# rossumur/espflix

Measured on AMD Instinct MI355X. Metric: MPEG-1 352x192 frames/s, higher is better.
Workload: dtype u8/int32; 1 GPU; 1024 streams/GPU x GOP(12) I+11P, 352x192 MPEG-1 ES resident in HBM, ids rank*1024.. per rank (BASELINE configs[2]; at 8 GPUs = configs[4], stream k on rank floor(k*8/8192)); streams_per_gpu=1024, streams_total=1024, es_bytes_per_gpu=46457181, parallelism=stream-partition x1, coefficients_per_gpu=44531885, ring_depth=2

## Files before the change

espflix_amd/csrc/efx_api.hip:

```cpp
#include <hip/hip_runtime.h>

#include <algorithm>
#include <memory>
#include <mutex>
#include <thread>

#include <cstdio>
#include <cstdlib>
#include <cstring>
#include <string>
#include <vector>

#include "efx.h"
#include "efx_internal.h"
#include "enc_core.h"
#include "parse_tm.h"

namespace efx {
struct DemuxChunk;
__global__ void k_demux_scan(const uint8_t*, const uint64_t*, const uint32_t*, const uint32_t*, DemuxChunk*);
__global__ void k_demux_offsets(const uint32_t*, const uint32_t*, DemuxChunk*, uint8_t*, const uint64_t*, uint32_t*, uint32_t*);
__global__ void k_demux(const uint8_t*, const uint64_t*, const uint32_t*, const uint32_t*, const DemuxChunk*, uint8_t*, PesEntry*);
__global__ void k_demux_fused(const uint8_t*, const uint64_t*, const uint32_t*, const uint32_t*, DemuxChunk*, uint8_t*, PesEntry*, uint32_t*, uint32_t*,
                              uint32_t*);
__global__ void k_demux_audio_scan(const uint8_t*, const uint64_t*, const uint32_t*, const uint32_t*, DemuxChunk*);
__global__ void k_demux_audio_offsets(const uint32_t*, const uint32_t*, DemuxChunk*, uint32_t*);
__global__ void k_demux_audio(const uint8_t*, const uint64_t*, const uint32_t*, const uint32_t*, const DemuxChunk*, uint8_t*, const uint64_t*);
__global__ void k_ts_sequences(const uint8_t*, const uint64_t*, const uint32_t*, const uint32_t*, PesEntry*, IdxInfo*);
__global__ void k_idx_bins(const PesEntry*, const uint32_t*, const IdxInfo*, uint32_t, uint32_t*, size_t);
__global__ void k_index(const uint8_t*, const uint64_t*, int, PicInfo*, SliceTmp*, uint32_t*, uint32_t*, uint32_t*,
                        const uint32_t*, const PesEntry*, const uint32_t*, const uint32_t*, int64_t*, int64_t*, int, int, int);
__global__ void k_advance(StreamState*, const uint32_t*, int64_t*, const int64_t*, int, int, int, int32_t*);
__global__ void k_slice_scan(const PicInfo*, const uint32_t*, int, int, const uint32_t*, uint32_t*, DecodeCounters*);
__global__ void k_slice_emit(const PicInfo*, const SliceTmp*, const uint32_t*, const uint64_t*, const uint32_t*, int, int,
                             const uint32_t*, SliceDesc*, uint32_t*);
__global__ void k_parse(const uint8_t*, const SliceDesc*, DecodeCounters*, const TmTables*, MbRec*, TmU4*, uint32_t*, uint32_t*,
                        int, int);
__global__ void k_recon(const MbRec*, const uint32_t*, const uint32_t*, const uint32_t*, uint8_t*, int, int, int, const int32_t*, int, int);
__global__ void k_recon_all(const MbRec*, const uint32_t*, const uint32_t*, const uint32_t*, uint8_t*, int, int, int, const int32_t*, int, int,
                            int, uint32_t*, uint32_t*, int);

__global__ void k_frame_hash(const uint8_t*, int, uint64_t*);
__global__ void k_fill(uint32_t*, uint32_t, size_t);
__global__ void k_composite(const uint8_t*, const VideoTables*, const VideoLineTemplates*, FieldArgs, uint16_t*);
__global__ void k_pdm(const int16_t*, int, int, int32_t*, uint16_t*);
template <int FMT, int CHROMA>
__global__ void k_export(const uint8_t*, int, ExportArgs);
__global__ void k_enc_begin(EncArgs);
__global__ void k_enc_rows(EncArgs);
__global__ void k_enc_pack(EncArgs);
__global__ void k_sbc(const uint8_t*, size_t, int, int, SbcState*, const SbcTables*, int16_t*, size_t, uint32_t*, uint32_t*, int);
__global__ void k_sbc_frames(const uint8_t*, size_t, int, int, SbcFrameInfo*, uint32_t*, uint32_t*, SbcQueues*);
__global__ void k_sbc_plan(const SbcFrameInfo*, int, int, const SbcState*, SbcFramePlan*, uint32_t*, SbcQueues*, uint32_t*, int, int, uint32_t*,
                           uint32_t*, SbcExtraItem*, uint8_t*);
__global__ void k_sbc_par_stereo(const uint8_t*, size_t, int, int, const SbcState*, SbcState*, const SbcTables*, const SbcFrameInfo*, int16_t*,
                                 size_t, uint32_t*, int, SbcQueues*, const uint32_t*, int, const SbcExtraItem*, int);
__global__ void k_sbc_par_mono(const uint8_t*, size_t, int, int, const SbcState*, SbcState*, const SbcTables*, const SbcFrameInfo*, int16_t*,
                               size_t, uint32_t*, int, SbcQueues*, const uint32_t*, int, const SbcExtraItem*, int);
__global__ void k_sbc_gen(const uint8_t*, size_t, int, int, const SbcState*, SbcState*, const SbcTables*, const SbcFrameInfo*,
                          const SbcFramePlan*, int16_t*, size_t, int, SbcQueues*, const uint32_t*, int, const uint8_t*, int);
__global__ void k_sbc_finish(const uint8_t*, size_t, int, int, SbcState*, const SbcState*, const SbcTables*, int16_t*, size_t, uint32_t*,
                             uint32_t*, int, uint32_t*);
}

using namespace efx;

#ifndef EFX_SBC_WG_PER_CU
#define EFX_SBC_WG_PER_CU 4
#endif

#ifndef EFX_PARSE_STREAMS
#define EFX_PARSE_STREAMS 2
#endif
#ifndef EFX_SLOTS
#define EFX_SLOTS 3
#endif
constexpr int kParseStreams = EFX_PARSE_STREAMS;
constexpr int kMaxGroups = 16;
static_assert(kMaxGroups <= kExportMaxGroups, "k_export takes every reconstruction group of a call");
#ifndef EFX_RECON_MERGE
#define EFX_RECON_MERGE 1
#endif
constexpr int kReconMerge = EFX_RECON_MERGE;
#ifndef EFX_GROUP_STREAMS
#define EFX_GROUP_STREAMS 1024
#endif
// ... 19 lines not shown
    uint8_t* d_frames = nullptr;
    StreamState* d_state = nullptr;

    struct Upload {
        uint8_t* d_es = nullptr;
        uint64_t* d_stream_off = nullptr;
        uint32_t* d_stream_perm = nullptr;
        uint32_t* d_ts_len = nullptr;
        uint32_t* d_pkt_base = nullptr;
        uint32_t* d_es_len = nullptr;
        uint32_t* d_pes_count = nullptr;
        PesEntry* d_pes = nullptr;
        uint8_t* h_es = nullptr;
        uint8_t* h_meta = nullptr;
        std::vector<uint64_t> stream_off;
        std::vector<uint32_t> es_len;
        int n_streams = 0;
        int sort_groups = 1;
        size_t es_used = 0, ts_bytes = 0;
        bool ts_input = false, valid = false;
        hipEvent_t uploaded = nullptr;
        hipEvent_t last_read[kParseStreams] = {};
        hipEvent_t ev_demux[2] = {nullptr, nullptr};
        bool demux_timed = false;
    } up[kUploads];
    int cur_up = -1;
    struct Arena {
        uint8_t* base;
        size_t bytes;
        bool owned;
    };
    std::vector<Arena> arenas;
    hipStream_t copy_stream = nullptr;
    uint8_t* d_ts = nullptr;
    DemuxChunk* d_demux_chunks = nullptr;
    size_t pes_cap = 0;
    IdxInfo* d_idx_info = nullptr;
    uint64_t* d_ts_off = nullptr;
    uint32_t* d_idx_len = nullptr;
    uint32_t* d_idx_base = nullptr;
    PesEntry* d_idx_seq = nullptr;
    bool ts_ready = false;

    struct Slot {
        uint32_t* d_pic_count = nullptr;
        uint32_t* d_status = nullptr;
        DecodeCounters* d_counters = nullptr;
        MbRec* d_mbrecs = nullptr;
        TmU4* d_raw = nullptr;
        uint32_t* d_coefs = nullptr;
        PicInfo* d_pics = nullptr;
        SliceTmp* d_slices_tmp = nullptr;
        uint32_t* d_qtab = nullptr;
        uint32_t* d_slice_base = nullptr;
        SliceDesc* d_descs = nullptr;
        int64_t* d_pts = nullptr;
        int32_t* d_call_pos = nullptr;
        uint32_t* d_recon_sync = nullptr;
        hipEvent_t parse_done[kReconMerge] = {}, recon_done = nullptr, wrap_cleared = nullptr;
        int epoch = 0;
        int upload = 0;
    } slot[kSlots];
    struct TimingEvents {
        hipEvent_t ev[5] = {nullptr, nullptr, nullptr, nullptr, nullptr};
    };
    std::vector<TimingEvents> timing_ring;
    uint64_t timed_calls = 0;
    struct Group {
        int slot, first, count;
        int half0, halves;
    };
    Group groups[kMaxGroups];
    int n_groups = 0;
    hipEvent_t last_recon_done = nullptr;
    uint64_t recon_groups_unsynced = 0;
    int last_upload = 0;
    int last_n_streams = 0;
    bool last_ts_input = false;
    uint64_t subcalls = 0;
    uint64_t parse_calls = 0;
    uint8_t timing_groups[kTimingRing] = {};
    uint16_t timing_launches[kTimingRing] = {};
    uint16_t timing_leaders[kTimingRing] = {};
    hipStream_t parse_streams[kParseStreams] = {};
    VideoTables* d_video[2] = {nullptr, nullptr};
    VideoLineTemplates* d_video_lines[2] = {nullptr, nullptr};
    SbcTables* d_sbc_tables = nullptr;
    int parse_wg_cap = 0;
    int opt_groups = 0;
    int opt_parse_cap = 0;
    int opt_recon_mode = 0;
    int opt_recon_waves = 0;
    int opt_recon_items = 16;
    int n_cus = 256;
    uint32_t* d_sbc_flags = nullptr;
    SbcState* d_sbc_next = nullptr;
    size_t sbc_flags_cap = 0;
    SbcFrameInfo* d_sbc_info = nullptr;
    SbcFramePlan* d_sbc_plan = nullptr;
    SbcExtraItem* d_sbc_extra = nullptr;
    uint8_t* d_sbc_cover = nullptr;
    size_t sbc_info_cap = 0;
    size_t sbc_gran_cap = 0;
    int opt_sbc_serial = 0;
    int opt_demux_fused = 0;
    bool sbc_flags_clean = false;
    uint64_t* d_hash = nullptr;
// ... 256 lines not shown
        int lo = 0, hi = 0;
        if (hipDeviceGetStreamPriorityRange(&lo, &hi) != hipSuccess)
            return bail(EFX_ERR_DEVICE);
        for (auto& ps : ctx->parse_streams)
            if (hipStreamCreateWithPriority(&ps, hipStreamNonBlocking, hi) != hipSuccess)
                return bail(EFX_ERR_DEVICE);
        if (hipStreamCreateWithFlags(&ctx->copy_stream, hipStreamNonBlocking) != hipSuccess)
            return bail(EFX_ERR_DEVICE);
        std::vector<hipStream_t> order = {ctx->stream};
        for (auto ps : ctx->parse_streams)
            order.push_back(ps);
        order.push_back(ctx->copy_stream);
        for (hipStream_t st : order) {
            hipLaunchKernelGGL(k_fill, dim3(1), dim3(64), 0, st, (uint32_t*)nullptr, 0u, (size_t)0);
            if (hipStreamSynchronize(st) != hipSuccess)
                return bail(EFX_ERR_DEVICE);
        }
    }
    const size_t n = (size_t)cfg->max_streams, P = (size_t)cfg->max_pictures, D = (size_t)ctx->cfg.ring_depth;
    ctx->es_cap = ctx->cfg.max_stream_bytes + n * (kEsTailBytes + 32) + kEsGuardBytes;
    ctx->es_cap = (ctx->es_cap + 255) & ~(size_t)255;
    if (ctx->es_cap * kCoefsPerEsByte >= 0xFFFFFFFFull)
        return bail(EFX_ERR_CAPACITY);
    hipError_t e = hipSuccess;
    auto A = [&](hipError_t r) {
        if (e == hipSuccess)
            e = r;
    };
    A(dalloc(&ctx->d_tables, 1));
    A(dalloc(&ctx->d_tm_tables, 1));
    A(dalloc(&ctx->d_state, n));
    for (auto& u : ctx->up) {
        A(dalloc(&u.d_es, ctx->es_cap));
        A(dalloc(&u.d_stream_off, n + 1));
        A(dalloc(&u.d_stream_perm, n));
        A(hipHostMalloc(reinterpret_cast<void**>(&u.h_es), ctx->es_cap, hipHostMallocDefault));
        A(hipHostMalloc(reinterpret_cast<void**>(&u.h_meta), meta_bytes(n), hipHostMallocDefault));
        A(hipEventCreateWithFlags(&u.uploaded, hipEventDisableTiming));
        for (auto& ev : u.last_read)
            A(hipEventCreateWithFlags(&ev, hipEventDisableTiming));
        if (e == hipSuccess)
            A(hipMemset(u.d_es, 0, ctx->es_cap));
    }
    for (auto& sl : ctx->slot) {
        A(dalloc(&sl.d_pic_count, n));
        A(dalloc(&sl.d_status, n));
        A(dalloc(&sl.d_counters, kMaxGroups));
        A(dalloc(&sl.d_mbrecs, n * P * kMbCount));
        A(dalloc(&sl.d_raw, n * P * kMbCount));
        A(dalloc(&sl.d_coefs, ctx->es_cap * kCoefsPerEsByte));
        A(dalloc(&sl.d_pics, n * P));
        A(dalloc(&sl.d_slices_tmp, n * P * kMaxSlicesPerPicture));
        A(dalloc(&sl.d_qtab, n * P * 64));
        A(dalloc(&sl.d_slice_base, n * P + kMaxGroups));
        A(dalloc(&sl.d_descs, n * P * kMaxSlicesPerPicture));
        A(dalloc(&sl.d_call_pos, 2 * n));
        A(dalloc(&sl.d_recon_sync, kReconSyncWords(n)));
    }
    A(dalloc(&ctx->d_frames, n * D * kFrameBytes + 8192));
    A(dalloc(&ctx->d_video[0], 1));
    A(dalloc(&ctx->d_video[1], 1));
    A(dalloc(&ctx->d_video_lines[0], 1));
    A(dalloc(&ctx->d_video_lines[1], 1));
    A(dalloc(&ctx->d_hash, n * D));
    A(dalloc(&ctx->d_sbc_tables, 1));
    if (e != hipSuccess) {
        fprintf(stderr, "efx_create: %s\n", hipGetErrorString(e));
        return bail(EFX_ERR_DEVICE);
    }
    {
        hipDeviceProp_t prop;
        if (hipGetDeviceProperties(&prop, cfg->device) == hipSuccess) {
            ctx->parse_wg_cap = std::max(1, prop.multiProcessorCount * 5 / 8);
            ctx->n_cus = std::max(1, prop.multiProcessorCount);
        }
        if (const char* v = getenv("EFX_GROUPS"))
            ctx->opt_groups = atoi(v);
        if (const char* v = getenv("EFX_FORCE_PARSE_CAP"))
            ctx->opt_parse_cap = atoi(v);
        if (const char* v = getenv("EFX_RECON_MODE"))
            ctx->opt_recon_mode = atoi(v);
        if (const char* v = getenv("EFX_RECON_WAVES"))
            ctx->opt_recon_waves = atoi(v);
        if (const char* v = getenv("EFX_DEMUX_FUSED"))
            ctx->opt_demux_fused = atoi(v) != 0;
        if (const char* v = getenv("EFX_RECON_ITEMS"))
            ctx->opt_recon_items = atoi(v);
        if (const char* cap = getenv("EFX_PARSE_WG_CAP"))
            ctx->parse_wg_cap = atoi(cap);
    }
    ParseTables* pt = new ParseTables;
    build_parse_tables(pt);
    A(hipMemcpy(ctx->d_tables, pt, sizeof(ParseTables), hipMemcpyHostToDevice));
    {
        TmTables* tt = new TmTables;
        build_tm_tables(tt);
        hipError_t e_tm = hipMemcpy(ctx->d_tm_tables, tt, sizeof(TmTables), hipMemcpyHostToDevice);
        delete tt;
        A(e_tm);
    }
    delete pt;
    for (int ntsc = 0; ntsc < 2; ntsc++) {
        VideoTables vt;
        build_video_tables(ntsc, &vt);
        A(hipMemcpy(ctx->d_video[ntsc], &vt, sizeof(vt), hipMemcpyHostToDevice));
        VideoLineTemplates* lt = new VideoLineTemplates;
        build_video_line_templates(&vt, lt);
// ... 23 lines not shown
    return EFX_OK;
}

void efx_destroy(efx_ctx* ctx)
{
    bind_device(ctx);
    if (!ctx)
        return;
    if (ctx->copy_stream)
        (void)hipStreamSynchronize(ctx->copy_stream);
    for (auto ps : ctx->parse_streams)
        if (ps)
            (void)hipStreamSynchronize(ps);
    if (ctx->stream)
        (void)hipStreamSynchronize(ctx->stream);
    for (auto& a : ctx->arenas) {
        if (a.owned)
            (void)hipHostFree(a.base);
        else
            (void)hipHostUnregister(a.base);
    }
    void* bufs[] = {ctx->d_tables, ctx->d_tm_tables, ctx->d_sbc_flags, ctx->d_sbc_next, ctx->d_sbc_info, ctx->d_sbc_plan, ctx->d_sbc_extra, ctx->d_sbc_cover, ctx->d_state, ctx->d_frames, ctx->d_video[0],  ctx->d_video[1], ctx->d_video_lines[0],
                    ctx->d_video_lines[1], ctx->d_hash, ctx->d_ts, ctx->d_demux_chunks, ctx->d_sbc_tables, ctx->d_idx_info, ctx->d_ts_off, ctx->d_idx_len,
                    ctx->d_idx_base, ctx->d_idx_seq, ctx->d_enc_state, ctx->d_enc_pics, ctx->d_enc_slices, ctx->d_enc_slice_len,
                    ctx->d_enc_tables};
    if (ctx->h_enc_full)
        (void)hipHostFree(ctx->h_enc_full);
    for (auto& te : ctx->timing_ring)
        for (auto& ev : te.ev)
            if (ev)
                (void)hipEventDestroy(ev);
    for (void* b : bufs)
        if (b)
            (void)dev_free(b);
    for (auto& u : ctx->up) {
        void* ub[] = {u.d_es, u.d_stream_off, u.d_stream_perm, u.d_ts_len, u.d_pkt_base, u.d_es_len, u.d_pes_count, u.d_pes};
        for (void* b : ub)
            if (b)
                (void)dev_free(b);
        if (u.h_es)
            (void)hipHostFree(u.h_es);
        if (u.h_meta)
            (void)hipHostFree(u.h_meta);
        hipEvent_t evs[] = {u.uploaded, u.ev_demux[0], u.ev_demux[1]};
        for (auto ev : evs)
            if (ev)
                (void)hipEventDestroy(ev);
        for (auto ev : u.last_read)
            if (ev)
                (void)hipEventDestroy(ev);
    }
    for (auto& sl : ctx->slot) {
        void* sb[] = {sl.d_pic_count, sl.d_status, sl.d_counters, sl.d_mbrecs, sl.d_raw, sl.d_coefs, sl.d_pts, sl.d_call_pos, sl.d_recon_sync,
                      sl.d_pics,      sl.d_slices_tmp, sl.d_qtab, sl.d_slice_base, sl.d_descs};
        for (void* b : sb)
            if (b)
                (void)dev_free(b);
        for (auto ev : sl.parse_done)
            if (ev)
                (void)hipEventDestroy(ev);
        if (sl.recon_done)
            (void)hipEventDestroy(sl.recon_done);
        if (sl.wrap_cleared)
            (void)hipEventDestroy(sl.wrap_cleared);
    }
    bool complete = ctx->own_stream && ctx->stream && ctx->copy_stream;
    for (auto ps : ctx->parse_streams)
        complete = complete && ps;
    if (ctx->pooled_streams && complete) {
        StreamSet set;
        set.recon = ctx->stream;
        for (int i = 0; i < kParseStreams; i++)
            set.parse[i] = ctx->parse_streams[i];
        set.copy = ctx->copy_stream;
        set.serial = ctx->stream_serial;
        park_stream_set(ctx->cfg.device, set);
    } else {
        for (auto ps : ctx->parse_streams)
            if (ps)
                (void)hipStreamDestroy(ps);
        if (ctx->copy_stream)
            (void)hipStreamDestroy(ctx->copy_stream);
        if (ctx->own_stream && ctx->stream)
            (void)hipStreamDestroy(ctx->stream);
    }
    delete ctx;
}


static int ensure_ts_buffers(efx_ctx* ctx)
{
    if (ctx->ts_ready)
        return EFX_OK;
    if (ctx->d_ts)
        return fail(ctx, EFX_ERR_DEVICE, "transport-stream buffers: an earlier allocation failed");
    const size_t n_max = (size_t)ctx->cfg.max_streams;
    ctx->pes_cap = ctx->es_cap / 188 + n_max;
    hipError_t e = dalloc(&ctx->d_ts, ctx->es_cap);
    if (e == hipSuccess)
        e = dev_alloc(reinterpret_cast<void**>(&ctx->d_demux_chunks), (ctx->pes_cap / kDemuxChunk + n_max + 2) * 16 + n_max * sizeof(uint32_t));
    for (auto& u : ctx->up) {
        if (e == hipSuccess) e = dalloc(&u.d_ts_len, n_max);
        if (e == hipSuccess) e = dalloc(&u.d_pkt_base, n_max);
        if (e == hipSuccess) e = dalloc(&u.d_es_len, n_max);
        if (e == hipSuccess) e = dalloc(&u.d_pes_count, n_max);
        if (e == hipSuccess) e = dalloc(&u.d_pes, ctx->pes_cap);
        for (auto& ev : u.ev_demux)
// ... 454 lines not shown
                                      : (idle_at_call ? group_count(n_all) : 1);
    {
        bool nested = true;
        for (int g = 1; g < G && nested; g++) {
            bool found = false;
            for (int k = 0; k <= u.sort_groups && !found; k++)
                found = group_first(n_all, u.sort_groups, k) == group_first(n_all, G, g);
            nested = found;
        }
        if (!nested) {
            int r = sync_all(ctx);
            if (r)
                return r;
            std::vector<uint32_t> perm((size_t)n_all);
            for (int i = 0; i < n_all; i++)
                perm[i] = (uint32_t)i;
            auto len_of = [&](uint32_t i) { return u.stream_off[i + 1] - u.stream_off[i]; };
            for (int g = 0; g < G; g++)
                std::stable_sort(perm.begin() + group_first(n_all, G, g), perm.begin() + group_first(n_all, G, g + 1),
                                 [&](uint32_t a, uint32_t b) { return len_of(a) > len_of(b); });
            EFX_HIP(hipMemcpy(u.d_stream_perm, perm.data(), perm.size() * sizeof(uint32_t), hipMemcpyHostToDevice));
            u.sort_groups = G;
        }
    }
    hipStream_t sr = ctx->stream;
    int timing_slot = -1;
    if (ctx->timing && !ctx->timing_ring.empty()) {
        timing_slot = (int)(ctx->timed_calls++ % kTimingRing);
        ctx->timing_groups[timing_slot] = (uint8_t)G;
        ctx->timing_leaders[timing_slot] = 0;
        ctx->timing_launches[timing_slot] = (uint16_t)(((G + kReconMerge - 1) / kReconMerge) * (ctx->opt_recon_mode == 0 ? n_pictures : 1));
    }
    ctx->last_upload = ctx->cur_up;
    ctx->last_n_streams = u.n_streams;
    ctx->last_ts_input = u.ts_input;
    const int R = (G + kReconMerge - 1) / kReconMerge;
    ctx->n_groups = R;
    for (int r = 0; r < R; r++) {
        const int h0 = r * kReconMerge, h1 = std::min(G, h0 + kReconMerge);
        const int rs0 = group_first(n_all, G, h0), rn = group_first(n_all, G, h1) - rs0;
        const int slot = (int)(ctx->subcalls++ % kSlots);
        ctx->groups[r] = {slot, rs0, rn, h0, h1 - h0};
        efx_ctx::Slot& sl = ctx->slot[slot];
        sl.upload = ctx->cur_up;
        const bool wrap = ++sl.epoch > 255;
        if (wrap)
            sl.epoch = 1;
        efx_ctx::TimingEvents* te0 = nullptr;
        for (int g = h0; g < h1; g++) {
            const int s0 = group_first(n_all, G, g), n = group_first(n_all, G, g + 1) - s0;
            const int pi = (int)(ctx->parse_calls++ % kParseStreams);
            hipStream_t sp = ctx->parse_streams[pi];
            DecodeCounters* counters = sl.d_counters + g;
            uint32_t* slice_base = sl.d_slice_base + (size_t)s0 * P + g;
            SliceDesc* descs = sl.d_descs + (size_t)s0 * P * kMaxSlicesPerPicture;

            EFX_HIP(hipStreamWaitEvent(sp, u.uploaded, 0));
            EFX_HIP(hipStreamWaitEvent(sp, sl.recon_done, 0));
            if (wrap && g == h0) {
                EFX_HIP(hipMemsetAsync(sl.d_mbrecs, 0, (size_t)ctx->cfg.max_streams * P * kMbCount * sizeof(MbRec), sp));
                EFX_HIP(hipEventRecord(sl.wrap_cleared, sp));
            } else if (wrap)
                EFX_HIP(hipStreamWaitEvent(sp, sl.wrap_cleared, 0));
            efx_ctx::TimingEvents* te = timing_slot >= 0 ? &ctx->timing_ring[(size_t)timing_slot * kMaxGroups + g] : nullptr;
            if (te && !te->ev[0])
                for (auto& ev : te->ev)
                    EFX_HIP(hipEventCreate(&ev));
            if (g == h0)
                te0 = te;
            if (te)
                EFX_HIP(hipEventRecord(te->ev[0], sp));
            hipLaunchKernelGGL(k_index, dim3(n), dim3(64 * kIndexWaves), 0, sp, u.d_es, u.d_stream_off, P, sl.d_pics, sl.d_slices_tmp,
                               sl.d_pic_count, sl.d_status, sl.d_qtab, ctx->d_tables->scan, u.d_pes, u.d_pkt_base, u.d_pes_count,
                               u.ts_input ? sl.d_pts : nullptr, u.ts_input ? sl.d_pts + (size_t)ctx->cfg.max_streams * P : nullptr,
                               first_picture, s0, n_pictures);
            hipLaunchKernelGGL(k_slice_scan, dim3(1), dim3(1024), 0, sp, sl.d_pics, sl.d_pic_count, n, P, u.d_stream_perm + s0,
                               slice_base, counters);
            hipLaunchKernelGGL(k_slice_emit, dim3((n * P * kMaxSlicesPerPicture + 255) / 256), dim3(256), 0, sp, sl.d_pics,
                               sl.d_slices_tmp, sl.d_pic_count, u.d_stream_off, slice_base, n, P, u.d_stream_perm + s0, descs, sl.d_status);
            if (te)
                EFX_HIP(hipEventRecord(te->ev[1], sp));
            const int max_slices = n * P * kMaxSlicesPerPicture;
            const int parse_waves = (max_slices + kParseLanes - 1) / kParseLanes;
            int parse_wgs = (parse_waves + kParseWaves - 1) / kParseWaves;
            const bool recon_busy = ctx->opt_parse_cap == 1 || (ctx->opt_parse_cap == 0 && ctx->recon_groups_unsynced > 0);
            if (ctx->parse_wg_cap > 0 && recon_busy)
                parse_wgs = std::min(parse_wgs, ctx->parse_wg_cap);
            hipLaunchKernelGGL(k_parse, dim3(parse_wgs), dim3(64 * kParseWaves), 0, sp, u.d_es,
                               descs, counters, ctx->d_tm_tables, sl.d_mbrecs, sl.d_raw, sl.d_coefs, sl.d_status, P, sl.epoch);
            if (te)
                EFX_HIP(hipEventRecord(te->ev[2], sp));
            EFX_HIP(hipEventRecord(sl.parse_done[g - h0], sp));
            EFX_HIP(hipEventRecord(u.last_read[pi], sp));
        }

        for (int g = h0; g < h1; g++)
            EFX_HIP(hipStreamWaitEvent(sr, sl.parse_done[g - h0], 0));
        if (te0) {
            EFX_HIP(hipEventRecord(te0->ev[4], sr));
            ctx->timing_leaders[timing_slot] |= (uint16_t)(1u << h0);
        }
        hipLaunchKernelGGL(k_advance, dim3((rn + 255) / 256), dim3(256), 0, sr, ctx->d_state, sl.d_pic_count,
                           u.ts_input ? sl.d_pts : nullptr, u.ts_input ? sl.d_pts + (size_t)ctx->cfg.max_streams * P : nullptr, rs0, rn,
                           P, sl.d_call_pos);
        constexpr int kGroupsPerPicture = (kMbCount * 6 + 63) / 64;
#ifdef EFX_RECON_ITEMS2
        constexpr int kReconGridY = (kGroupsPerPicture + 1) / 2;
#else
        constexpr int kReconGridY = kGroupsPerPicture;
#endif
        if (ctx->opt_recon_mode == 0) {
            for (int p = 0; p < n_pictures; p++)
                hipLaunchKernelGGL(k_recon, dim3(rn, kReconGridY), dim3(64), 0, sr, sl.d_mbrecs, sl.d_coefs,
                                   ctx->d_tables->scan, sl.d_qtab, ctx->d_frames, P, D, p, sl.d_call_pos, sl.epoch, rs0);
        } else if (rn > 0) {
            EFX_HIP(hipMemsetAsync(sl.d_recon_sync, 0, kReconSyncWords((size_t)rn) * sizeof(uint32_t), sr));
            const long long items = (long long)rn * kGroupsPerPicture * n_pictures;
            const int per_cu = ctx->opt_recon_waves > 0 ? ctx->opt_recon_waves : 18;
            const long long waves = ctx->opt_recon_items > 0 ? (items + ctx->opt_recon_items - 1) / ctx->opt_recon_items
                                                             : std::min<long long>(items, (long long)ctx->n_cus * per_cu);
            hipLaunchKernelGGL(k_recon_all, dim3((unsigned)waves), dim3(64), 0, sr, sl.d_mbrecs,
                               sl.d_coefs, ctx->d_tables->scan, sl.d_qtab, ctx->d_frames, P, D, n_pictures, sl.d_call_pos, sl.epoch, rs0, rn,
                               sl.d_recon_sync, sl.d_status, ctx->opt_recon_items);
        }
        if (te0)
            EFX_HIP(hipEventRecord(te0->ev[3], sr));
        EFX_HIP(hipEventRecord(sl.recon_done, sr));
        ctx->last_recon_done = sl.recon_done;
        ctx->recon_groups_unsynced++;
    }
    EFX_HIP(hipGetLastError());
    ctx->decoded = true;
// ... 787 lines not shown
            float a = 0, b = 0, c = 0;
            EFX_HIP(hipEventElapsedTime(&a, te.ev[0], te.ev[1]));
            EFX_HIP(hipEventElapsedTime(&b, te.ev[1], te.ev[2]));
            if (leaders >> g & 1) {
                EFX_HIP(hipEventElapsedTime(&c, te.ev[4], te.ev[3]));
                last_leader = g;
                n_leaders++;
            }
            t.index_ms += a / n_timed;
            t.parse_ms += b / n_timed;
            t.recon_ms += c / n_timed;
        }
        float d = 0;
        EFX_HIP(hipEventElapsedTime(&d, ctx->timing_ring[call * kMaxGroups].ev[0], ctx->timing_ring[call * kMaxGroups + last_leader].ev[3]));
        t.total_ms += d / n_timed;
        if (k == 0) {
            t.groups = (uint32_t)n_leaders;
            t.parse_halves = (uint32_t)G;
            t.recon_launches = ctx->timing_launches[call];
        } else if (t.groups != (uint32_t)n_leaders || t.parse_halves != (uint32_t)G || t.recon_launches != ctx->timing_launches[call])
            t.mixed = 1;
    }
    t.timed_calls = (uint32_t)n_timed;
    for (int i = 0; i < ctx->n_streams; i++)
        t.pictures += ctx->h_pic_count[i];
    t.slices = ctx->h_counters.total_slices;
    t.coefficients = ctx->h_counters.coefficients;
    {
        efx_ctx::Upload& u = ctx->up[ctx->last_upload];
        t.es_bytes = u.es_used;
        t.ts_bytes = u.ts_bytes;
        if (u.ts_input && u.demux_timed)
            EFX_HIP(hipEventElapsedTime(&t.demux_ms, u.ev_demux[0], u.ev_demux[1]));
    }
    *out = t;
    return EFX_OK;
}


int efx_debug_poke(efx_ctx* ctx, void* dptr, size_t bytes, long long offset_bytes)
{
    bind_device(ctx);
    if (!ctx || !dptr)
        return EFX_ERR_ARG;
    (void)bytes;
    char* at = static_cast<char*>(dptr) + offset_bytes;
    hipLaunchKernelGGL(k_fill, dim3(1), dim3(64), 0, ctx->stream, reinterpret_cast<uint32_t*>(at), 0xDEADBEEFu, (size_t)1);
    EFX_HIP(hipGetLastError());
    EFX_HIP(hipStreamSynchronize(ctx->stream));
    ctx->recon_groups_unsynced = 0;
    return EFX_OK;
}

int efx_debug_recon_stats(efx_ctx* ctx, uint32_t out[64])
{
    bind_device(ctx);
    if (!ctx || !out || !ctx->decoded || ctx->n_groups < 1)
        return EFX_ERR_ARG;
    int r = sync_all(ctx);
    if (r)
        return r;
    std::vector<uint32_t> all(64 * 32);
    EFX_HIP(hipMemcpy(all.data(), ctx->slot[ctx->groups[ctx->n_groups - 1].slot].d_recon_sync, all.size() * sizeof(uint32_t), hipMemcpyDeviceToHost));
    for (int k = 0; k < 64; k++)
        out[k] = all[(size_t)k * 32];
    return EFX_OK;
}

int efx_device_alloc(efx_ctx* ctx, size_t bytes, void** dptr)
{
    bind_device(ctx);
    if (!ctx || !dptr)
        return EFX_ERR_ARG;
    EFX_HIP(dev_alloc(dptr, bytes));
    return EFX_OK;
}

int efx_device_free(efx_ctx* ctx, void* dptr)
{
    bind_device(ctx);
    if (!ctx)
        return EFX_ERR_ARG;
    EFX_HIP(dev_free(dptr));
    return EFX_OK;
}

int efx_memcpy_h2d(efx_ctx* ctx, void* dst_device, const void* src, size_t bytes)
{
    bind_device(ctx);
    if (!ctx || !dst_device || !src)
        return EFX_ERR_ARG;
    EFX_HIP(hipStreamSynchronize(ctx->stream));
    ctx->recon_groups_unsynced = 0;
    EFX_HIP(hipMemcpy(dst_device, src, bytes, hipMemcpyHostToDevice));
    return EFX_OK;
}

int efx_memcpy_d2h(efx_ctx* ctx, void* dst, const void* src_device, size_t bytes)
{
    bind_device(ctx);
    if (!ctx || !dst || !src_device)
        return EFX_ERR_ARG;
    EFX_HIP(hipStreamSynchronize(ctx->stream));
    ctx->recon_groups_unsynced = 0;
    EFX_HIP(hipMemcpy(dst, src_device, bytes, hipMemcpyDeviceToHost));
    return EFX_OK;
// ... 4 lines not shown
```

espflix_amd/csrc/efx_internal.h:

```cpp
#pragma once
#include <cstdint>

namespace efx {

constexpr int kMbW = 22, kMbH = 12, kMbCount = 264;
constexpr int kStride = 528, kStripBytes = 8448, kFrameBytes = 101376;
constexpr int kMaxSlicesPerPicture = 16;
#ifndef EFX_PARSE_LANES
#define EFX_PARSE_LANES 64
#endif
constexpr int kParseLanes = EFX_PARSE_LANES;
#ifndef EFX_PARSE_WAVES
#define EFX_PARSE_WAVES 4
#endif
constexpr int kParseWaves = EFX_PARSE_WAVES;
constexpr int kIndexWaves = 4;
constexpr int kMaxUnitsPerStream = 4096;
constexpr int kCoefsPerEsByte = 4;
constexpr int kEsTailBytes = 9;
constexpr int kEsGuardBytes = 512;

struct PicInfo {
    uint32_t first_slice;
    uint16_t n_slices;
    uint8_t type;
    uint8_t full_pel;
    uint8_t r_size;
    uint8_t custom_q;
    uint16_t reserved;
    uint32_t seq_off;
    uint32_t start_off;
};

struct PesEntry {
    uint32_t es_off;
    uint32_t reserved;
    int64_t pts;
};

struct StreamState {
    uint32_t fb_index;
    uint32_t pts_seen;
    int64_t pts_carry;
};

constexpr int64_t kNoPts = INT64_MIN;

struct SliceTmp {
    uint32_t off;
    uint32_t len_code;
};

struct SliceDesc {
    uint32_t es_off;
    uint32_t es_len;
    uint32_t stream;
    uint32_t pic_code_flags;
    uint32_t mb_limit;
    uint32_t reserved;
};
// ... 170 lines not shown
```

espflix_amd/csrc/k_index.hip:

```cpp
#include <hip/hip_runtime.h>

#include "efx_internal.h"
#include "efx.h"

namespace efx {

namespace {

__device__ inline uint32_t wave_excl_scan(uint32_t v, uint32_t* total)
{
    uint32_t x = v;
    int lane = threadIdx.x & 63;
#pragma unroll
    for (int d = 1; d < 64; d <<= 1) {
        uint32_t y = __shfl_up(x, d, 64);
        if (lane >= d)
            x += y;
    }
    *total = __shfl(x, 63, 64);
    return x - v;
}

__device__ inline uint32_t load_bits(const uint8_t* p, uint32_t bitpos, int n)
{
// ... 316 lines not shown
            }
            pts_out[(size_t)s * max_pictures + p] = a ? mp[a - 1].pts : -1;
        }
    }

    for (uint32_t p = wave; p < npics; p += kIndexWaves) {
        PicInfo pi = mypics[p];
        if (!pi.custom_q)
            continue;
        uint32_t flags = pi.reserved;
        const uint8_t* sp = base + pi.seq_off;
        uint32_t intra_bit = 63, non_intra_bit = (flags & 1) ? 64 + 512 : 64;
        uint32_t t = scan_tab[lane];
        uint32_t zz = t & 0xFF;
        uint32_t qi = (flags & 1) ? load_bits(sp, intra_bit + 8 * zz, 8) : ((t >> 16) & 0xFF);
        uint32_t qn = (flags & 2) ? load_bits(sp, non_intra_bit + 8 * zz, 8) : 16;
        qtab[((size_t)s * max_pictures + p) * 64 + lane] = (t & 0xFFFF) | (qi << 16) | (qn << 24);
    }
}

__global__ void k_advance(StreamState* __restrict__ state, const uint32_t* __restrict__ pic_count, int64_t* __restrict__ pts,
                          const int64_t* __restrict__ pts_newest, int stream0, int n_streams, int max_pictures,
                          int32_t* __restrict__ call_pos)
{
    const int t = blockIdx.x * blockDim.x + threadIdx.x;
    if (t >= n_streams)
        return;
    const int s = stream0 + t;
    StreamState st = state[s];
    const int n = (int)pic_count[s];
    int f = st.pts_seen ? -1 : n;
    if (pts) {
        int64_t* my = pts + (size_t)s * max_pictures;
        for (int i = 0; i < n; i++) {
            if (my[i] == -1 && st.pts_carry != -1)
                my[i] = st.pts_carry;
            if (f == n && my[i] != -1)
                f = i;
        }
        if (pts_newest[s] != kNoPts)
            st.pts_carry = pts_newest[s];
    } else if (!st.pts_seen)
        f = 0;
    call_pos[2 * s] = (int32_t)st.fb_index;
    call_pos[2 * s + 1] = f;
    if (n > 0) {
        st.fb_index += f < 0 ? (uint32_t)n : (uint32_t)(n - 1 > f ? n - 1 - f : 0);
        if (f < n)
            st.pts_seen = 1;
    }
    state[s] = st;
}

__global__ __launch_bounds__(1024) void k_slice_scan(const PicInfo* __restrict__ pics,
                                                     const uint32_t* __restrict__ pic_count, int n_streams,
                                                     int max_pictures, const uint32_t* __restrict__ stream_perm,
                                                     uint32_t* __restrict__ slice_base,
                                                     DecodeCounters* __restrict__ counters)
{
    __shared__ uint32_t wave_tot[16];
    __shared__ uint32_t carry;
    constexpr int kRun = 4;
    const int tid = threadIdx.x, lane = tid & 63, wv = tid >> 6;
    const int n = n_streams * max_pictures;
    if (tid == 0)
        carry = 0;
    __syncthreads();
    for (int base = 0; base < n; base += 1024 * kRun) {
        uint32_t v[kRun];
#pragma unroll
        for (int r = 0; r < kRun; r++) {
            const int i = base + tid * kRun + r;
            v[r] = 0;
            if (i < n) {
                int p = i / n_streams, s = (int)stream_perm[i - p * n_streams];
                if ((uint32_t)p < pic_count[s])
                    v[r] = pics[(size_t)s * max_pictures + p].n_slices;
            }
        }
        uint32_t mine = 0;
#pragma unroll
        for (int r = 0; r < kRun; r++)
            mine += v[r];
        uint32_t tot;
        uint32_t ex = wave_excl_scan(mine, &tot);
        if (lane == 63)
            wave_tot[wv] = tot;
        __syncthreads();
        uint32_t off = carry;
        for (int k = 0; k < wv; k++)
            off += wave_tot[k];
        uint32_t at = off + ex;
#pragma unroll
        for (int r = 0; r < kRun; r++) {
            const int i = base + tid * kRun + r;
            if (i < n)
                slice_base[i] = at;
            at += v[r];
        }
        __syncthreads();
        if (tid == 1023)
            carry = at;
        __syncthreads();
    }
    if (tid == 0) {
        counters->total_slices = carry;
        counters->streams = (uint32_t)n_streams;
        counters->coefficients = 0;
        counters->macroblocks = 0;
        counters->next_wave = 0;
        slice_base[n] = carry;
    }
}

__global__ __launch_bounds__(256) void k_slice_emit(const PicInfo* __restrict__ pics,
                                                    const SliceTmp* __restrict__ slices_tmp,
                                                    const uint32_t* __restrict__ pic_count,
                                                    const uint64_t* __restrict__ stream_off,
                                                    const uint32_t* __restrict__ slice_base, int n_streams,
                                                    int max_pictures, const uint32_t* __restrict__ stream_perm,
                                                    SliceDesc* __restrict__ descs, uint32_t* __restrict__ status)
{
    int t = blockIdx.x * blockDim.x + threadIdx.x;
    int k = t % kMaxSlicesPerPicture, i = t / kMaxSlicesPerPicture;
    if (i >= n_streams * max_pictures)
        return;
    int p = i / n_streams, s = (int)stream_perm[i - p * n_streams];
    if ((uint32_t)p >= pic_count[s])
        return;
    PicInfo pi = pics[(size_t)s * max_pictures + p];
    if (k >= pi.n_slices)
        return;
    SliceTmp st = slices_tmp[(size_t)s * max_pictures * kMaxSlicesPerPicture + pi.first_slice + k];
    SliceDesc d;
    d.es_off = (uint32_t)stream_off[s] + st.off;
    d.es_len = st.len_code >> 8;
    d.stream = (uint32_t)s;
    d.pic_code_flags = (uint32_t)p | ((st.len_code & 0xFF) << 8) | ((uint32_t)pi.type << 16) | ((uint32_t)pi.full_pel << 18) |
                       ((uint32_t)pi.r_size << 19) | ((uint32_t)pi.custom_q << 22);
    uint32_t limit = kMbCount;
    bool out_of_order = false;
    {
        const uint32_t code = st.len_code & 0xFF;
        const SliceTmp* all = slices_tmp + (size_t)s * max_pictures * kMaxSlicesPerPicture + pi.first_slice;
        for (int j = 0; j < (int)pi.n_slices; j++) {
            const uint32_t other = all[j].len_code & 0xFF;
            if (other > code && (other - 1) * kMbW < limit)
                limit = (other - 1) * kMbW;
            if (other == code && j > k)
                limit = 0;
            out_of_order |= j < k && other >= code;
        }
    }
    if (out_of_order)
        atomicOr(&status[s], EFX_STREAM_SLICE_ORDER);
    d.mb_limit = limit;
    d.reserved = 0;
    descs[slice_base[i] + k] = d;
}

}
```

espflix_amd/csrc/k_parse.hip:

```cpp
#include <hip/hip_runtime.h>

#include "efx_internal.h"
#include "efx.h"
#include "parse_tm.h"
#include "efx_probe.h"

namespace efx {

namespace {

constexpr int kRingDwords = 16;
#ifndef EFX_TRIPS_PER_TOPUP
#define EFX_TRIPS_PER_TOPUP 4
#endif
constexpr int kTripsPerTopup = EFX_TRIPS_PER_TOPUP;
constexpr int kRingLow = kTripsPerTopup + 4;
#ifndef EFX_DRAIN_WORDS
#define EFX_DRAIN_WORDS 4
#endif
constexpr int kDrainWords = EFX_DRAIN_WORDS;
constexpr int kStageWords = (kTripsPerTopup <= 4 && kDrainWords == 4) ? 8 : 16;

struct BitReader {
    const uint4* gp;
// ... 123 lines not shown
__device__ __forceinline__ void parse_group(uint32_t w, const uint8_t* __restrict__ es, const SliceDesc* __restrict__ descs,
                                            DecodeCounters* __restrict__ counters, SharedTables& sh, MbRec* __restrict__ mbrecs,
                                            TmU4* __restrict__ raw_recs, uint32_t* __restrict__ coefs, uint32_t* __restrict__ status,
                                            int max_pictures, int epoch)
{
    const uint32_t gid = w * kParseLanes + (threadIdx.x & 63);
    const bool mine = (threadIdx.x & 63) < kParseLanes && gid < counters->total_slices;
    SliceDesc d = {};
    if (mine)
        d = descs[gid];
    const uint32_t pic = d.pic_code_flags & 0xFF;
    EFX_PROBE_CLAIM(1, w);
    EFX_PROBE_STAMP(1);
    const int code = (d.pic_code_flags >> 8) & 0xFF;
    const int first_mb = (code - 1) * kMbW;
    const int mb_limit = (int)d.mb_limit;
    const bool has_slice = mine && mb_limit > first_mb;

    TmSlice sp;
    sp.coef_last = (d.es_off + d.es_len) * kCoefsPerEsByte - 1;
    sp.type_bit = ((d.pic_code_flags >> 16) & 3) == 1 ? kTmTypeIBit : 0u;
    sp.r_size = (d.pic_code_flags >> 19) & 7;
    sp.max_mbs = has_slice ? (uint32_t)(mb_limit - first_mb) : 0u;
    const size_t rec0 = ((size_t)d.stream * max_pictures + pic) * kMbCount;
    TmU4* const raw = raw_recs + rec0 + (has_slice ? first_mb : 0);

    BitReader br;
    br.init(es, d.es_off, &sh.ring[threadIdx.x >> 6][0][threadIdx.x & 63]);

    TmFix fx;
    {
        fx.qscale = br.window() >> 27;
        br.advance(5);
        while (has_slice && (br.window() >> 31)) {
            br.advance(9);
            br.topup();
        }
        br.advance(1);
    }
    TmLane L;
    const uint32_t tok_base = d.es_off * kCoefsPerEsByte;
    tm_begin(L, tok_base, has_slice);
    auto store_raw = [&](uint32_t k, uint32_t a, uint32_t b, uint32_t c, uint32_t e) { raw[k] = make_uint4(a, b, c, e); };
    const char* const tab = reinterpret_cast<const char*>(&sh.t);
    StageSink sink{&sh.stage[threadIdx.x >> 6][0][threadIdx.x & 63], coefs, sp.coef_last, d.es_off * kCoefsPerEsByte};
    auto lookup = [&](uint32_t st, uint32_t win) {
        return *reinterpret_cast<const TmE*>(tab + (st >> 16) + ((win >> (st & 31)) << 3));
    };

    EFX_PROBE_STAMP(2);
    EFX_PROBE_SET(6, pic | ((d.pic_code_flags >> 16) & 3) << 8);
    static_assert(kTripsPerTopup + 3 <= kRingLow && kRingLow <= kRingDwords - 4, "the window reads two dwords ahead; a top-up adds whole groups of four");
#ifdef EFX_PROBE
    unsigned efx_probe_trips = 0;
#endif
    uint32_t win = br.window();
    TmE e = lookup(L.st, win);
    do {
        br.topup();
        sink.drain(L.tok);
        if (__any(tm_guard(L))) {
            win = br.window();
            e = lookup(L.st, win);
        }
#pragma unroll
        for (int t = 0; t < kTripsPerTopup; t++) {
            const uint32_t win0 = win;
            const TmE e0 = e;
            const bool overflow = tm_trip(
                L, win0, e0, sp,
                [&](uint32_t bits, uint32_t st) {
                    br.advance(bits);
                    win = br.window();
                    e = lookup(st, win);
                },
                sink, store_raw);
            if (__any(overflow)) {
                if (overflow) {
                    br.back(tm_overflow(L, e0, sp, sink, store_raw));
                    win = br.window();
                    e = lookup(L.st, win);
                }
            }
        }
#ifdef EFX_PROBE
        efx_probe_trips += kTripsPerTopup;
#endif
    } while (__any(tm_alive(L.st)));
    EFX_PROBE_STAMP(3);
    EFX_PROBE_SET(5, efx_probe_trips);
    if (!has_slice)
        return;
    sink.finish(L.tok);
    tm_end(L, sp, store_raw);

    fx.code = code;
    fx.mb_limit = mb_limit;
    fx.full_pel = (d.pic_code_flags >> 18) & 1;
    fx.r_size = sp.r_size;
    fx.rec_flags = ((d.pic_code_flags >> 22) & 1) ? 0x80u : 0u;
    fx.epoch = (uint32_t)epoch;
    fx.coef_last = sp.coef_last;
    uint32_t n_mbs = 0, n_coefs = 0;
    uint32_t st = tm_finish(L, fx, tok_base, [&](uint32_t k) { return raw[k]; }, coefs, reinterpret_cast<TmU4*>(mbrecs + rec0),
                            &n_mbs, &n_coefs);
    if (br.pos - (d.es_off & 15) * 8 > d.es_len * 8 + kTmEndBits)
        st |= EFX_STREAM_BAD_VLC;
    if (tm_why(L.st) == kDeadEnd) {
        const uint8_t* unit = es + d.es_off - (d.es_off & 15);
        const uint32_t end = (d.es_off & 15) + d.es_len;
        uint32_t at = br.pos >> 3;
        bool junk = false;
        if (at < end) {
            junk = (unit[at] & (0xFFu >> (br.pos & 7))) != 0;
            for (at++; at < end && !junk; at++)
                junk = unit[at] != 0;
        }
        if (junk)
            st |= EFX_STREAM_SERIAL_HUNT;
    }
    EFX_PROBE_MAX(4, wall_clock64());
    if (st)
        atomicOr(&status[d.stream], st);
    atomicAdd(&counters->coefficients, (unsigned long long)n_coefs);
    atomicAdd(&counters->macroblocks, (unsigned long long)n_mbs);
}

__global__ __launch_bounds__(64 * kParseWaves) void k_parse(const uint8_t* __restrict__ es, const SliceDesc* __restrict__ descs,
                                                            DecodeCounters* __restrict__ counters,
                                                            const TmTables* __restrict__ gtab, MbRec* __restrict__ mbrecs,
                                                            TmU4* __restrict__ raw_recs, uint32_t* __restrict__ coefs,
                                                            uint32_t* __restrict__ status, int max_pictures, int epoch)
{
    const uint32_t n_groups = (counters->total_slices + kParseLanes - 1) / kParseLanes;
    if (blockIdx.x * kParseWaves >= n_groups)
        return;
    __builtin_amdgcn_s_setprio(3);
    __shared__ SharedTables sh;
    {
        const uint4* src = reinterpret_cast<const uint4*>(gtab);
        uint4* dst = reinterpret_cast<uint4*>(&sh.t);
        for (int i = threadIdx.x; i < (int)(sizeof(TmTables) / 16); i += blockDim.x)
            dst[i] = src[i];
// ... 17 lines not shown
```

Before: 9.018 million frames/s.

## Sort slice descriptors by length class so parse waves get similar-length slices

Replaces the per-picture slice prefix scan with a block histogram over log-spaced slice-length classes, a global scan over the class counts, and a ranked scatter. Descriptors end up grouped by length, longest first, with dead slices (duplicate codes) placed in a final class. The goal is to cut lane divergence in the wavefront-wide parse loop, which runs until the longest slice in a wave finishes, and to schedule long slices early. In exchange there is an extra kernel launch, repeated slot computation in both count and emit, and slices from the same stream no longer sit next to each other, which may hurt locality.

```diff
diff --git a/espflix_amd/csrc/efx_api.hip b/espflix_amd/csrc/efx_api.hip
--- a/espflix_amd/csrc/efx_api.hip
+++ b/espflix_amd/csrc/efx_api.hip
@@ -31,7 +31,8 @@
 __global__ void k_index(const uint8_t*, const uint64_t*, int, PicInfo*, SliceTmp*, uint32_t*, uint32_t*, uint32_t*,
                         const uint32_t*, const PesEntry*, const uint32_t*, const uint32_t*, int64_t*, int64_t*, int, int, int);
 __global__ void k_advance(StreamState*, const uint32_t*, int64_t*, const int64_t*, int, int, int, int32_t*);
-__global__ void k_slice_scan(const PicInfo*, const uint32_t*, int, int, const uint32_t*, uint32_t*, DecodeCounters*);
+__global__ void k_slice_count(const PicInfo*, const SliceTmp*, const uint32_t*, int, int, const uint32_t*, uint32_t*);
+__global__ void k_slice_scan(uint32_t*, int, int, DecodeCounters*);
 __global__ void k_slice_emit(const PicInfo*, const SliceTmp*, const uint32_t*, const uint64_t*, const uint32_t*, int, int,
                              const uint32_t*, SliceDesc*, uint32_t*);
 __global__ void k_parse(const uint8_t*, const SliceDesc*, DecodeCounters*, const TmTables*, MbRec*, TmU4*, uint32_t*, uint32_t*,
@@ -157,7 +158,7 @@
         PicInfo* d_pics = nullptr;
         SliceTmp* d_slices_tmp = nullptr;
         uint32_t* d_qtab = nullptr;
-        uint32_t* d_slice_base = nullptr;
+        uint32_t* d_slice_class = nullptr;
         SliceDesc* d_descs = nullptr;
         int64_t* d_pts = nullptr;
         int32_t* d_call_pos = nullptr;
@@ -520,7 +521,7 @@
         A(dalloc(&sl.d_pics, n * P));
         A(dalloc(&sl.d_slices_tmp, n * P * kMaxSlicesPerPicture));
         A(dalloc(&sl.d_qtab, n * P * 64));
-        A(dalloc(&sl.d_slice_base, n * P + kMaxGroups));
+        A(dalloc(&sl.d_slice_class, ((n * P * kMaxSlicesPerPicture + kSliceBlock - 1) / kSliceBlock + kMaxGroups) * kSliceClasses));
         A(dalloc(&sl.d_descs, n * P * kMaxSlicesPerPicture));
         A(dalloc(&sl.d_call_pos, 2 * n));
         A(dalloc(&sl.d_recon_sync, kReconSyncWords(n)));
@@ -650,7 +651,7 @@
     }
     for (auto& sl : ctx->slot) {
         void* sb[] = {sl.d_pic_count, sl.d_status, sl.d_counters, sl.d_mbrecs, sl.d_raw, sl.d_coefs, sl.d_pts, sl.d_call_pos, sl.d_recon_sync,
-                      sl.d_pics,      sl.d_slices_tmp, sl.d_qtab, sl.d_slice_base, sl.d_descs};
+                      sl.d_pics,      sl.d_slices_tmp, sl.d_qtab, sl.d_slice_class, sl.d_descs};
         for (void* b : sb)
             if (b)
                 (void)dev_free(b);
@@ -1211,7 +1212,8 @@
             const int pi = (int)(ctx->parse_calls++ % kParseStreams);
             hipStream_t sp = ctx->parse_streams[pi];
             DecodeCounters* counters = sl.d_counters + g;
-            uint32_t* slice_base = sl.d_slice_base + (size_t)s0 * P + g;
+            uint32_t* class_base = sl.d_slice_class + ((size_t)s0 * P * kMaxSlicesPerPicture / kSliceBlock + g) * kSliceClasses;
+            const int slice_blocks = (n * P * kMaxSlicesPerPicture + kSliceBlock - 1) / kSliceBlock;
             SliceDesc* descs = sl.d_descs + (size_t)s0 * P * kMaxSlicesPerPicture;
 
             EFX_HIP(hipStreamWaitEvent(sp, u.uploaded, 0));
@@ -1233,10 +1235,11 @@
                                sl.d_pic_count, sl.d_status, sl.d_qtab, ctx->d_tables->scan, u.d_pes, u.d_pkt_base, u.d_pes_count,
                                u.ts_input ? sl.d_pts : nullptr, u.ts_input ? sl.d_pts + (size_t)ctx->cfg.max_streams * P : nullptr,
                                first_picture, s0, n_pictures);
-            hipLaunchKernelGGL(k_slice_scan, dim3(1), dim3(1024), 0, sp, sl.d_pics, sl.d_pic_count, n, P, u.d_stream_perm + s0,
-                               slice_base, counters);
-            hipLaunchKernelGGL(k_slice_emit, dim3((n * P * kMaxSlicesPerPicture + 255) / 256), dim3(256), 0, sp, sl.d_pics,
-                               sl.d_slices_tmp, sl.d_pic_count, u.d_stream_off, slice_base, n, P, u.d_stream_perm + s0, descs, sl.d_status);
+            hipLaunchKernelGGL(k_slice_count, dim3(slice_blocks), dim3(kSliceBlock), 0, sp, sl.d_pics, sl.d_slices_tmp, sl.d_pic_count, n, P,
+                               u.d_stream_perm + s0, class_base);
+            hipLaunchKernelGGL(k_slice_scan, dim3(1), dim3(1024), 0, sp, class_base, slice_blocks, n, counters);
+            hipLaunchKernelGGL(k_slice_emit, dim3(slice_blocks), dim3(kSliceBlock), 0, sp, sl.d_pics, sl.d_slices_tmp, sl.d_pic_count,
+                               u.d_stream_off, class_base, n, P, u.d_stream_perm + s0, descs, sl.d_status);
             if (te)
                 EFX_HIP(hipEventRecord(te->ev[1], sp));
             const int max_slices = n * P * kMaxSlicesPerPicture;
@@ -2130,6 +2133,31 @@
     return EFX_OK;
 }
 
+#ifdef EFX_PROBE
+int efx_probe_read_slices(efx_ctx* ctx, int half, uint32_t* dst, size_t max_slices)
+{
+    bind_device(ctx);
+    if (!ctx || !dst || !ctx->decoded || ctx->n_groups < 1 || half < 0)
+        return EFX_ERR_ARG;
+    if (sync_all(ctx))
+        return EFX_ERR_DEVICE;
+    const efx_ctx::Group& lastg = ctx->groups[ctx->n_groups - 1];
+    const int G = lastg.half0 + lastg.halves;
+    if (half >= G)
+        return EFX_ERR_ARG;
+    const efx_ctx::Slot& sl = ctx->slot[ctx->groups[half / kReconMerge].slot];
+    const int s0 = group_first(ctx->last_n_streams, G, half);
+    DecodeCounters c;
+    if (hipMemcpy(&c, sl.d_counters + half, sizeof(c), hipMemcpyDeviceToHost) != hipSuccess)
+        return EFX_ERR_DEVICE;
+    const size_t n = std::min<size_t>(c.total_slices, max_slices);
+    static_assert(sizeof(SliceDesc) == 24, "six words per descriptor");
+    if (hipMemcpy(dst, sl.d_descs + (size_t)s0 * ctx->cfg.max_pictures * kMaxSlicesPerPicture, n * sizeof(SliceDesc), hipMemcpyDeviceToHost) != hipSuccess)
+        return EFX_ERR_DEVICE;
+    return (int)c.total_slices;
+}
+#endif
+
 int efx_debug_recon_stats(efx_ctx* ctx, uint32_t out[64])
 {
     bind_device(ctx);
diff --git a/espflix_amd/csrc/efx_internal.h b/espflix_amd/csrc/efx_internal.h
--- a/espflix_amd/csrc/efx_internal.h
+++ b/espflix_amd/csrc/efx_internal.h
@@ -6,6 +6,10 @@
 constexpr int kMbW = 22, kMbH = 12, kMbCount = 264;
 constexpr int kStride = 528, kStripBytes = 8448, kFrameBytes = 101376;
 constexpr int kMaxSlicesPerPicture = 16;
+constexpr int kSliceLenClasses = 32;
+constexpr int kSliceClassMinLog = 5;
+constexpr int kSliceClasses = kSliceLenClasses + 1;
+constexpr int kSliceBlock = 1024;
 #ifndef EFX_PARSE_LANES
 #define EFX_PARSE_LANES 64
 #endif
diff --git a/espflix_amd/csrc/k_index.hip b/espflix_amd/csrc/k_index.hip
--- a/espflix_amd/csrc/k_index.hip
+++ b/espflix_amd/csrc/k_index.hip
@@ -392,17 +392,86 @@
     state[s] = st;
 }
 
-__global__ __launch_bounds__(1024) void k_slice_scan(const PicInfo* __restrict__ pics,
-                                                     const uint32_t* __restrict__ pic_count, int n_streams,
-                                                     int max_pictures, const uint32_t* __restrict__ stream_perm,
-                                                     uint32_t* __restrict__ slice_base,
+static_assert(kSliceBlock % kMaxSlicesPerPicture == 0 && kSliceBlock / 64 <= 16, "whole pictures per block, at most 16 waves");
+
+namespace {
+
+__device__ inline uint32_t slice_class(uint32_t bytes)
+{
+    const uint32_t v = bytes < (1u << kSliceClassMinLog) ? (1u << kSliceClassMinLog) : bytes;
+    const uint32_t e = 31u - (uint32_t)__clz((int)v);
+    const uint32_t q = ((e - kSliceClassMinLog) << 2) | ((v >> (e - 2)) & 3u);
+    return (uint32_t)(kSliceLenClasses - 1) - (q < (uint32_t)kSliceLenClasses ? q : (uint32_t)(kSliceLenClasses - 1));
+}
+
+struct SliceSlot {
+    int s, p, k;
+    PicInfo pi;
+    SliceTmp st;
+    const SliceTmp* all;
+    uint32_t cls;
+};
+
+__device__ inline bool slice_slot(int t, const PicInfo* __restrict__ pics, const SliceTmp* __restrict__ slices_tmp,
+                                  const uint32_t* __restrict__ pic_count, int n_streams, int max_pictures,
+                                  const uint32_t* __restrict__ stream_perm, SliceSlot& o)
+{
+    o.k = t % kMaxSlicesPerPicture;
+    const int i = t / kMaxSlicesPerPicture;
+    if (i >= n_streams * max_pictures)
+        return false;
+    o.p = i / n_streams;
+    o.s = (int)stream_perm[i - o.p * n_streams];
+    if ((uint32_t)o.p >= pic_count[o.s])
+        return false;
+    o.pi = pics[(size_t)o.s * max_pictures + o.p];
+    if (o.k >= o.pi.n_slices)
+        return false;
+    o.all = slices_tmp + (size_t)o.s * max_pictures * kMaxSlicesPerPicture + o.pi.first_slice;
+    o.st = o.all[o.k];
+    o.cls = slice_class(o.st.len_code >> 8);
+    for (int j = o.k + 1; j < (int)o.pi.n_slices; j++)
+        if ((o.all[j].len_code & 0xFF) == (o.st.len_code & 0xFF))
+            o.cls = kSliceLenClasses;
+    return true;
+}
+
+}
+
+__global__ __launch_bounds__(kSliceBlock) void k_slice_count(const PicInfo* __restrict__ pics,
+                                                             const SliceTmp* __restrict__ slices_tmp,
+                                                             const uint32_t* __restrict__ pic_count, int n_streams,
+                                                             int max_pictures, const uint32_t* __restrict__ stream_perm,
+                                                             uint32_t* __restrict__ class_base)
+{
+    __shared__ uint32_t hist[kSliceClasses];
+    const int tid = threadIdx.x;
+    if (tid < kSliceClasses)
+        hist[tid] = 0;
+    __syncthreads();
+    SliceSlot o;
+    const bool have = slice_slot((int)blockIdx.x * kSliceBlock + tid, pics, slices_tmp, pic_count, n_streams, max_pictures,
+                                 stream_perm, o);
+    for (unsigned long long todo = __ballot(have); todo;) {
+        const uint32_t c = (uint32_t)__shfl((int)o.cls, __ffsll((long long)todo) - 1, 64);
+        const unsigned long long m = __ballot(have && o.cls == c);
+        if ((tid & 63) == 0)
+            atomicAdd(&hist[c], (uint32_t)__popcll(m));
+        todo &= ~m;
+    }
+    __syncthreads();
+    if (tid < kSliceClasses)
+        class_base[tid * (int)gridDim.x + (int)blockIdx.x] = hist[tid];
+}
+
+__global__ __launch_bounds__(1024) void k_slice_scan(uint32_t* __restrict__ class_base, int n_blocks, int n_streams,
                                                      DecodeCounters* __restrict__ counters)
 {
     __shared__ uint32_t wave_tot[16];
     __shared__ uint32_t carry;
     constexpr int kRun = 4;
     const int tid = threadIdx.x, lane = tid & 63, wv = tid >> 6;
-    const int n = n_streams * max_pictures;
+    const int n = kSliceClasses * n_blocks;
     if (tid == 0)
         carry = 0;
     __syncthreads();
@@ -411,12 +480,7 @@
 #pragma unroll
         for (int r = 0; r < kRun; r++) {
             const int i = base + tid * kRun + r;
-            v[r] = 0;
-            if (i < n) {
-                int p = i / n_streams, s = (int)stream_perm[i - p * n_streams];
-                if ((uint32_t)p < pic_count[s])
-                    v[r] = pics[(size_t)s * max_pictures + p].n_slices;
-            }
+            v[r] = i < n ? class_base[i] : 0u;
         }
         uint32_t mine = 0;
 #pragma unroll
@@ -435,7 +499,7 @@
         for (int r = 0; r < kRun; r++) {
             const int i = base + tid * kRun + r;
             if (i < n)
-                slice_base[i] = at;
+                class_base[i] = at;
             at += v[r];
         }
         __syncthreads();
@@ -449,54 +513,68 @@
         counters->coefficients = 0;
         counters->macroblocks = 0;
         counters->next_wave = 0;
-        slice_base[n] = carry;
-    }
-}
-
-__global__ __launch_bounds__(256) void k_slice_emit(const PicInfo* __restrict__ pics,
-                                                    const SliceTmp* __restrict__ slices_tmp,
-                                                    const uint32_t* __restrict__ pic_count,
-                                                    const uint64_t* __restrict__ stream_off,
-                                                    const uint32_t* __restrict__ slice_base, int n_streams,
-                                                    int max_pictures, const uint32_t* __restrict__ stream_perm,
-                                                    SliceDesc* __restrict__ descs, uint32_t* __restrict__ status)
-{
-    int t = blockIdx.x * blockDim.x + threadIdx.x;
-    int k = t % kMaxSlicesPerPicture, i = t / kMaxSlicesPerPicture;
-    if (i >= n_streams * max_pictures)
+    }
+}
+
+__global__ __launch_bounds__(kSliceBlock) void k_slice_emit(const PicInfo* __restrict__ pics,
+                                                            const SliceTmp* __restrict__ slices_tmp,
+                                                            const uint32_t* __restrict__ pic_count,
+                                                            const uint64_t* __restrict__ stream_off,
+                                                            const uint32_t* __restrict__ class_base, int n_streams,
+                                                            int max_pictures, const uint32_t* __restrict__ stream_perm,
+                                                            SliceDesc* __restrict__ descs, uint32_t* __restrict__ status)
+{
+    __shared__ uint32_t wave_cnt[kSliceBlock / 64][kSliceClasses];
+    const int tid = threadIdx.x, lane = tid & 63, wv = tid >> 6;
+    for (int i = tid; i < (kSliceBlock / 64) * kSliceClasses; i += kSliceBlock)
+        (&wave_cnt[0][0])[i] = 0;
+    __syncthreads();
+    SliceSlot o;
+    const bool have = slice_slot((int)blockIdx.x * kSliceBlock + tid, pics, slices_tmp, pic_count, n_streams, max_pictures,
+                                 stream_perm, o);
+    uint32_t rank = 0;
+    for (unsigned long long todo = __ballot(have); todo;) {
+        const uint32_t c = (uint32_t)__shfl((int)o.cls, __ffsll((long long)todo) - 1, 64);
+        const unsigned long long m = __ballot(have && o.cls == c);
+        if (have && o.cls == c)
+            rank = (uint32_t)__popcll(m & ((1ull << lane) - 1));
+        if (lane == 0)
+            wave_cnt[wv][c] = (uint32_t)__popcll(m);
+        todo &= ~m;
+    }
+    __syncthreads();
+    if (!have)
         return;
-    int p = i / n_streams, s = (int)stream_perm[i - p * n_streams];
-    if ((uint32_t)p >= pic_count[s])
-        return;
-    PicInfo pi = pics[(size_t)s * max_pictures + p];
-    if (k >= pi.n_slices)
-        return;
-    SliceTmp st = slices_tmp[(size_t)s * max_pictures * kMaxSlicesPerPicture + pi.first_slice + k];
+    const int s = o.s;
+    const PicInfo pi = o.pi;
+    const SliceTmp st = o.st;
     SliceDesc d;
     d.es_off = (uint32_t)stream_off[s] + st.off;
     d.es_len = st.len_code >> 8;
     d.stream = (uint32_t)s;
-    d.pic_code_flags = (uint32_t)p | ((st.len_code & 0xFF) << 8) | ((uint32_t)pi.type << 16) | ((uint32_t)pi.full_pel << 18) |
+    d.pic_code_flags = (uint32_t)o.p | ((st.len_code & 0xFF) << 8) | ((uint32_t)pi.type << 16) | ((uint32_t)pi.full_pel << 18) |
                        ((uint32_t)pi.r_size << 19) | ((uint32_t)pi.custom_q << 22);
     uint32_t limit = kMbCount;
     bool out_of_order = false;
     {
         const uint32_t code = st.len_code & 0xFF;
-        const SliceTmp* all = slices_tmp + (size_t)s * max_pictures * kMaxSlicesPerPicture + pi.first_slice;
         for (int j = 0; j < (int)pi.n_slices; j++) {
-            const uint32_t other = all[j].len_code & 0xFF;
+            const uint32_t other = o.all[j].len_code & 0xFF;
             if (other > code && (other - 1) * kMbW < limit)
                 limit = (other - 1) * kMbW;
-            if (other == code && j > k)
-                limit = 0;
-            out_of_order |= j < k && other >= code;
-        }
-    }
+            out_of_order |= j < o.k && other >= code;
+        }
+    }
+    if (o.cls == (uint32_t)kSliceLenClasses)
+        limit = 0;
     if (out_of_order)
         atomicOr(&status[s], EFX_STREAM_SLICE_ORDER);
     d.mb_limit = limit;
     d.reserved = 0;
-    descs[slice_base[i] + k] = d;
-}
-
-}
+    uint32_t at = class_base[o.cls * (uint32_t)gridDim.x + blockIdx.x] + rank;
+    for (int w = 0; w < wv; w++)
+        at += wave_cnt[w][o.cls];
+    descs[at] = d;
+}
+
+}
diff --git a/espflix_amd/csrc/k_parse.hip b/espflix_amd/csrc/k_parse.hip
--- a/espflix_amd/csrc/k_parse.hip
+++ b/espflix_amd/csrc/k_parse.hip
@@ -199,11 +199,14 @@
     EFX_PROBE_SET(6, pic | ((d.pic_code_flags >> 16) & 3) << 8);
     static_assert(kTripsPerTopup + 3 <= kRingLow && kRingLow <= kRingDwords - 4, "the window reads two dwords ahead; a top-up adds whole groups of four");
 #ifdef EFX_PROBE
-    unsigned efx_probe_trips = 0;
+    unsigned efx_probe_trips = 0, efx_probe_live = 0;
 #endif
     uint32_t win = br.window();
     TmE e = lookup(L.st, win);
     do {
+#ifdef EFX_PROBE
+        efx_probe_live += (unsigned)__popcll(__ballot(tm_alive(L.st))) * kTripsPerTopup;
+#endif
         br.topup();
         sink.drain(L.tok);
         if (__any(tm_guard(L))) {
@@ -235,7 +238,7 @@
 #endif
     } while (__any(tm_alive(L.st)));
     EFX_PROBE_STAMP(3);
-    EFX_PROBE_SET(5, efx_probe_trips);
+    EFX_PROBE_SET(5, efx_probe_trips | (unsigned long long)efx_probe_live << 32);
     if (!has_slice)
         return;
     sink.finish(L.tok);
```

Result: faster. 9.299 million frames/s, median of 6 (+3.1%).
